# Arieys/MonteCarloPathTracing

Measured on AMD Instinct MI355X. Metric: Mrays/s on cornell-box 1280x720 SPP=256 (closest-hit queries actually traced / wall time incl. gather), higher is better.
Workload: dtype f64

## Files before the change

### montecarlopathtracing_amd/csrc/trace_pool.hpp

```cpp
#pragma once
#include "env.hpp"
#include "trace_persistent.hpp"
#include "vertex.hpp"

namespace mcpt {

struct NoPaths { static constexpr bool kPaths = false; };

#ifndef MCPT_POOL_WAVES
#define MCPT_POOL_WAVES 16
#endif
#ifndef MCPT_POOL_KT
#define MCPT_POOL_KT 20
#endif
#ifndef MCPT_POOL_STACK
#define MCPT_POOL_STACK 8
#endif
#define MCPT_POOL_SPILL (MCPT_FAST_STACK - MCPT_POOL_STACK)
#ifndef MCPT_POOL_CLAIMS
#define MCPT_POOL_CLAIMS 2
#endif
#define MCPT_POOL_CLAIM_ORDER __ATOMIC_ACQUIRE
#define MCPT_POOL_FILE_ORDER __ATOMIC_RELEASE

struct alignas(16) PoolOxy { double ox, oy; };
struct alignas(16) PoolOzDx { double oz, dx; };
struct alignas(16) PoolDyz { double dy, dz; };
struct alignas(16) PoolRcp { float rx, ry, rz, limit; };
typedef double pool_d2 __attribute__((ext_vector_type(2)));
template <class T>
__device__ __forceinline__ T pool_ld16(const T* p)
{
    static_assert(sizeof(T) == 16, "16-byte group");
    const pool_d2 v = *reinterpret_cast<const pool_d2*>(p);
    T r;
    __builtin_memcpy(&r, &v, 16);
    return r;
}

template <int NW, int KT, int SCAP>
struct PoolLds {
    PoolOxy oxy[KT * 64];
    PoolOzDx ozdx[KT * 64];
    PoolDyz dyz[KT * 64];
    PoolRcp rcp[KT * 64];
    double best_t[KT * 64];
    unsigned int q[KT * 64];
    int cur[KT * 64];
    int best_leaf[KT * 64];
    int spf[KT * 64];
    int stack[SCAP * KT * 64];
    unsigned int cls[5 * 64];
    unsigned int busy[64];
    int tbl[NW * 64];
    unsigned int stat[8];
    unsigned int live;
    unsigned int dry;
};

__device__ __forceinline__ int uni(int v) { return __builtin_amdgcn_readfirstlane(v); }
__device__ __forceinline__ long long uni(long long v)
{
    const int lo = __builtin_amdgcn_readfirstlane((int)(unsigned int)(unsigned long long)v);
    const int hi = __builtin_amdgcn_readfirstlane((int)(unsigned int)((unsigned long long)v >> 32));
    return (long long)(((unsigned long long)(unsigned int)hi << 32) | (unsigned int)lo);
}

template <class Src, int NW, int KT, int SCAP, class PP = NoPaths>
__device__ __forceinline__ void trace_pool(const DScene& S, const Src& src, TraceQueue* queue, long long* __restrict__ slow_list,
                                           unsigned int slow_cap, long long chunk, PoolLds<NW, KT, SCAP>& L, Work& w,
                                           int* __restrict__ spill ,
                                           const PP& pp = PP())
{
    static_assert(KT <= 32, "one 32-bit set per class");
    enum { C_INNER = 0, C_LEAF = 1, C_EXACT = 2, C_FIN = 3, C_SHADE = 4, C_DEAD = 5 };
    enum { F_FOUND = 256, F_AMBIG = 512, F_RAY = 1024, F_OWNFAIL = 2048  };
    const DFast& F = S.fast;
    const CwNode* __restrict__ nodes = F.cw;
    const DTri* __restrict__ tris = F.tris;
    const DTriPre* __restrict__ pre = F.pre;
    const TicketSchedule ts = make_ticket_schedule(src.total(), chunk);
    const int lane = threadIdx.x & 63, wave = uni((int)(threadIdx.x >> 6));
    const int stack_max = spill ? SCAP + MCPT_POOL_SPILL : SCAP;
    const int stack_cap = F.stack_cap < stack_max ? F.stack_cap : stack_max;
    int* __restrict__ my_spill = spill ? spill + (size_t)blockIdx.x * MCPT_POOL_SPILL * (KT * 64) : nullptr;
    auto st_put = [&](int e, int k, int v) __attribute__((always_inline)) {
        if (e < SCAP) L.stack[(e * KT + k) * 64 + lane] = v;
        else my_spill[((e - SCAP) * KT + k) * 64 + lane] = v;
    };
    auto st_get = [&](int e, int k) __attribute__((always_inline)) -> int {
        return e < SCAP ? L.stack[(e * KT + k) * 64 + lane] : my_spill[((e - SCAP) * KT + k) * 64 + lane];
    };

    for (int k = wave; k < KT; k += NW) { L.spf[k * 64 + lane] = 0; if constexpr (PP::kPaths) L.q[k * 64 + lane] = 0u; }
    int R = 1, NP = KT;
    if constexpr (PP::kPaths) { R = pp.nl + 1; NP = KT / R; }
    if (wave == 0) {
        L.cls[C_INNER * 64 + lane] = 0u; L.cls[C_LEAF * 64 + lane] = 0u; L.cls[C_EXACT * 64 + lane] = 0u;
        L.cls[C_FIN * 64 + lane] = PP::kPaths ? 0u : (unsigned int)((1ull << KT) - 1ull);
        L.cls[C_SHADE * 64 + lane] = PP::kPaths ? (unsigned int)((1ull << NP) - 1ull) : 0u;
        L.busy[lane] = 0u;
    }
    if (threadIdx.x == 0) { L.live = (PP::kPaths ? NP : KT) * 64; L.dry = 0; }
    if (threadIdx.x < 8) L.stat[threadIdx.x] = 0u;
    __syncthreads();

    unsigned int c_nodes = 0, c_rays = 0, c_exact = 0;
#ifdef MCPT_POOL_DEBUG
    unsigned long long d_used = 0, d_okc = 0, d_steps = 0, d_kill = 0, d_tickets = 0;
    unsigned long long d_cs[5] = {0, 0, 0, 0, 0}, d_cl[5] = {0, 0, 0, 0, 0}, d_sleep = 0, d_miss = 0, d_want[5] = {0, 0, 0, 0, 0};
    unsigned long long d_cyc[6] = {0, 0, 0, 0, 0, 0};
    unsigned long long d_t = __builtin_amdgcn_s_memtime();
    const unsigned long long d_t0 = d_t;
#endif
    long long next = 0, range_end = 0;
    bool queue_empty = false;
    int rot = wave % KT;
    const int rot_stride = (int)((0x13110d0bu >> (8 * ((wave >> 1) & 3))) & 255u) % KT | 1;
    const float s3f = __double2float_ru(3.0 * F.absmax), absmax_f = __double2float_ru(F.absmax);
    auto pad_of = [&](float of, float rf_) __attribute__((always_inline)) { return (0x1p-20f * 1.00001f) * ((fabsf(of) + s3f) * fabsf(rf_)); };
    auto margin_of = [&](const float of[3], const PoolRcp& a4) __attribute__((always_inline)) {
        const float rmax = fmaxf(fmaxf(fabsf(a4.rx), fabsf(a4.ry)), fabsf(a4.rz));
        const float scale = fmaxf(fmaxf(absmax_f, fabsf(of[0])), fmaxf(fabsf(of[1]), fabsf(of[2])));
        return rmax <= 0.99e6f ? (1.0000001e-9f * 1.00001f) * (scale * rmax) : __builtin_inff();
    };
    auto pop_next = [&](int idx, int k, int spf) __attribute__((always_inline)) -> int {
        int sp = spf & 255;
        if (sp == 0) return C_FIN;
        sp--;
        int nxt;
        if (!__ballot(sp >= SCAP)) { nxt = L.stack[(sp * KT + k) * 64 + lane]; __asm__ volatile("" : "+v"(nxt)); }
        else nxt = st_get(sp, k);
        const bool node = nxt >= 0;
        const int ref = -1 - nxt;
        const int first = node ? nxt : ref >> 4, cnt = (ref & 7) + 1;
        L.cur[idx] = first;
        L.spf[idx] = (spf & 0xff00) | sp | (node ? 0 : cnt << 16);
        return node ? C_INNER : C_LEAF;
    };

    for (;;) {
        const unsigned int m_inner = __hip_atomic_load(&L.cls[C_INNER * 64 + lane], __ATOMIC_RELAXED, __HIP_MEMORY_SCOPE_WORKGROUP);
        const unsigned int m_leaf = __hip_atomic_load(&L.cls[C_LEAF * 64 + lane], __ATOMIC_RELAXED, __HIP_MEMORY_SCOPE_WORKGROUP);
        const unsigned int m_exact = __hip_atomic_load(&L.cls[C_EXACT * 64 + lane], __ATOMIC_RELAXED, __HIP_MEMORY_SCOPE_WORKGROUP);
        const unsigned int m_fin = __hip_atomic_load(&L.cls[C_FIN * 64 + lane], __ATOMIC_RELAXED, __HIP_MEMORY_SCOPE_WORKGROUP);
        const int n_inner = __popcll(__ballot(m_inner != 0u));
        const int n_leaf = __popcll(__ballot(m_leaf != 0u));
        const int n_exact = __popcll(__ballot(m_exact != 0u));
        const bool fin_ok = PP::kPaths || !queue_empty || uni((int)__hip_atomic_load(&L.dry, __ATOMIC_RELAXED, __HIP_MEMORY_SCOPE_WORKGROUP)) == NW;
        const int n_fin = fin_ok ? __popcll(__ballot(m_fin != 0u)) : 0;
        unsigned int m_shade = 0u;
        int n_shade = 0;
        if constexpr (PP::kPaths) {
            m_shade = __hip_atomic_load(&L.cls[C_SHADE * 64 + lane], __ATOMIC_RELAXED, __HIP_MEMORY_SCOPE_WORKGROUP);
            n_shade = __popcll(__ballot(m_shade != 0u));
        }
        if (!(n_inner | n_leaf | n_exact | n_fin | n_shade)) {
            if (uni((int)__hip_atomic_load(&L.live, __ATOMIC_RELAXED, __HIP_MEMORY_SCOPE_WORKGROUP)) == 0) break;
            __builtin_amdgcn_s_sleep(4);
#ifdef MCPT_POOL_DEBUG
            d_sleep++;
#endif
            continue;
        }
        int c = C_FIN, best_score = n_fin;
        if (n_exact > best_score) { c = C_EXACT; best_score = n_exact; }
        if (n_leaf > best_score) { c = C_LEAF; best_score = n_leaf; }
        if (n_inner > best_score) { c = C_INNER; best_score = n_inner; }
        if (PP::kPaths && n_shade >= best_score && n_shade) { c = C_SHADE; best_score = n_shade; }
        c = uni(c);

        bool have = false;
        int k = 0;
        unsigned int cm = c == C_INNER ? m_inner : (c == C_LEAF ? m_leaf : (c == C_EXACT ? m_exact : (c == C_FIN ? m_fin : m_shade)));
        unsigned int* const cword = &L.cls[c * 64 + lane];
        const unsigned int below = 0xffffffffu >> (31 - rot), above = 0xffffffffu << rot;
#pragma unroll
        for (int attempt = 0; attempt < MCPT_POOL_CLAIMS; attempt++) {
            const bool want = !have && cm != 0u;
            if (attempt && !__ballot(want)) break;
            if (want) {
                int kk;
                if (wave & 1) { const unsigned int lo = cm & below; kk = 31 - __clz((int)(lo ? lo : cm)); }
                else { const unsigned int hi = cm & above; kk = __ffs((int)(hi ? hi : cm)) - 1; }
                const unsigned int bit = 1u << kk;
                const unsigned int old = __hip_atomic_fetch_and(cword, ~bit, MCPT_POOL_CLAIM_ORDER, __HIP_MEMORY_SCOPE_WORKGROUP);
                have = (old & bit) != 0u;
                k = kk;
                cm = old & ~bit;
            }
        }
        { rot += rot_stride; if (rot >= KT) rot -= KT; }
        const unsigned long long hv = __ballot(have);
#ifdef MCPT_POOL_DEBUG
        if (!hv) d_miss++;
#endif
        if (!hv) continue;
        const int n_have = __popcll(hv);
#ifdef MCPT_POOL_DEBUG
        { const unsigned long long tn = __builtin_amdgcn_s_memtime(); d_cyc[5] += tn - d_t; d_t = tn; }
        d_cs[c]++; d_cl[c] += n_have; d_want[c] += c == C_INNER ? n_inner : (c == C_LEAF ? n_leaf : (c == C_EXACT ? n_exact : (c == C_FIN ? n_fin : n_shade)));
#endif
        const int idx = k * 64 + lane;
        int nc = C_DEAD;
        __asm__ volatile("" ::: "memory");

        if (c == C_INNER) {
            bool refused = false;
            if (have) {
                const int cur = L.cur[idx];
                int spf = L.spf[idx];
                const PoolOxy a0 = pool_ld16(&L.oxy[idx]); const PoolOzDx a1 = pool_ld16(&L.ozdx[idx]); const PoolRcp a4 = L.rcp[idx];
                const float limit = a4.limit;
                RayF rf;
                rf.o[0] = (float)a0.ox; rf.o[1] = (float)a0.oy; rf.o[2] = (float)a1.oz;
                rf.r[0] = a4.rx; rf.r[1] = a4.ry; rf.r[2] = a4.rz;
                rf.pad[0] = pad_of(rf.o[0], a4.rx); rf.pad[1] = pad_of(rf.o[1], a4.ry); rf.pad[2] = pad_of(rf.o[2], a4.rz);
                int sp = spf & 255;
                if (sp > stack_cap - 3) {
                    L.spf[idx] = spf | F_AMBIG; nc = C_FIN; refused = true;
                } else {
                    const CwHits h = cw_step(nodes + cur, rf, limit);
                    const int n_hit = (h.ref[0] != MCPT_FAST_EMPTY) + (h.ref[1] != MCPT_FAST_EMPTY) + (h.ref[2] != MCPT_FAST_EMPTY) + (h.ref[3] != MCPT_FAST_EMPTY);
                    if (!__ballot(sp + n_hit - 1 > SCAP)) {
                        int* const col = &L.stack[k * 64 + lane];
                        if (n_hit >= 4) col[sp * (KT * 64)] = h.ref[3];
                        if (n_hit >= 3) col[(sp + n_hit - 3) * (KT * 64)] = h.ref[2];
                        if (n_hit >= 2) col[(sp + n_hit - 2) * (KT * 64)] = h.ref[1];
                        sp += n_hit > 1 ? n_hit - 1 : 0;
                    } else {
                        if (h.ref[3] != MCPT_FAST_EMPTY) { st_put(sp, k, h.ref[3]); sp++; }
                        if (h.ref[2] != MCPT_FAST_EMPTY) { st_put(sp, k, h.ref[2]); sp++; }
                        if (h.ref[1] != MCPT_FAST_EMPTY) { st_put(sp, k, h.ref[1]); sp++; }
                    }
                    int nxt = h.ref[0];
                    {
                        const bool pop = nxt == MCPT_FAST_EMPTY && sp > 0;
                        if (pop) sp--;
                        if (!__ballot(pop && sp >= SCAP)) { if (pop) { nxt = L.stack[(sp * KT + k) * 64 + lane]; __asm__ volatile("" : "+v"(nxt)); } }
                        else if (pop) nxt = st_get(sp, k);
                    }
                    const bool node = nxt >= 0, none = nxt == MCPT_FAST_EMPTY;
                    const int ref = -1 - nxt;
                    const int first = node ? nxt : ref >> 4, cnt = (ref & 7) + 1;
                    if (!none) L.cur[idx] = first;
                    spf = (spf & 0xff00) | sp | ((!node && !none) ? cnt << 16 : 0);
                    L.spf[idx] = spf;
                    nc = node ? C_INNER : (none ? C_FIN : C_LEAF);
                }
            }
            c_nodes += (unsigned int)(n_have - __popcll(__ballot(refused)));
        } else if (c == C_LEAF) {
            if (have) {
                const int cur = L.cur[idx];
                const int spf0 = L.spf[idx];
                const int cnt = (spf0 >> 16) & 255;
                const PoolOxy a0 = pool_ld16(&L.oxy[idx]); const PoolOzDx a1 = pool_ld16(&L.ozdx[idx]); const PoolDyz a2 = pool_ld16(&L.dyz[idx]); const PoolRcp a4 = L.rcp[idx];
                const float of[3] = {(float)a0.ox, (float)a0.oy, (float)a1.oz};
                const float limit = a4.limit, margin = margin_of(of, a4);
                unsigned int surv = 0;
                w.tris += cnt;
                if (!pre) surv = (1u << cnt) - 1u;
                else {
                    Ray r; r.o = mk(a0.ox, a0.oy, a1.oz); r.d = mk(a1.dx, a2.dy, a2.dz);
                    const PreRay pr = make_pre_ray(F, r, of, margin);
                    surv = leaf_survivors(pre, cur, cnt, pr, limit);
#ifdef MCPT_PRE_CHECK
                    const unsigned int wrong = leaf_wrongly_rejected(tris, cur, cnt, surv, r, (spf0 & F_FOUND) != 0, L.best_t[idx]);
                    w.pre_wrong += (unsigned int)__popc(wrong); surv |= wrong;
#endif
                }
                if (surv) { L.spf[idx] = (spf0 & 0xffff) | ((int)surv << 16); nc = C_EXACT; }
                else nc = pop_next(idx, k, spf0);
            }
        } else if (c == C_EXACT) {
            c_exact += (unsigned int)n_have;
            if (have) {
                const int cur = L.cur[idx];
                int spf = L.spf[idx];
                int surv = (spf >> 16) & 255;
                const PoolOxy a0 = pool_ld16(&L.oxy[idx]); const PoolOzDx a1 = pool_ld16(&L.ozdx[idx]); const PoolDyz a2 = pool_ld16(&L.dyz[idx]);
                const double best_t = L.best_t[idx];
                Ray r; r.o = mk(a0.ox, a0.oy, a1.oz); r.d = mk(a1.dx, a2.dy, a2.dz);
                const int kk = __ffs(surv) - 1;
                surv &= surv - 1;
                const int ti = cur + kk;
                const DTri* tr = tris + ti;
                const bool found = (spf & F_FOUND) != 0;
                V3 p;
                const bool hit = tri_hit(tr, r, p);
                if (hit) {
                    const double ta = (p.x - r.o.x) * fast_rcp(r.d.x);
                    if (ta > 0.0) {
                        const double band = best_t * 0x1p-47;
                        if (!found || ta < best_t - band) {
                            const PoolRcp a4 = L.rcp[idx];
                            const float of[3] = {(float)a0.ox, (float)a0.oy, (float)a1.oz};
                            L.best_t[idx] = ta; L.best_leaf[idx] = ti;
                            L.rcp[idx].limit = lead_limit(ta, margin_of(of, a4));
                            const bool own = own_box_hit(tr, r, mk(fast_rcp(r.d.x), fast_rcp(r.d.y), fast_rcp(r.d.z)));
                            spf = (spf & ~F_OWNFAIL) | F_FOUND | (own ? 0 : F_OWNFAIL);
                        } else if (!(ta > best_t + band)) {
                            const DTri* lt = tris + L.best_leaf[idx];
                            if (tie_prefers_new(r, p.x, hit_point(lt, r).x, tr, lt)) {
                                L.best_t[idx] = ta; L.best_leaf[idx] = ti;
                                const bool own = own_box_hit(tr, r, mk(fast_rcp(r.d.x), fast_rcp(r.d.y), fast_rcp(r.d.z)));
                                spf = (spf & ~F_OWNFAIL) | (own ? 0 : F_OWNFAIL);
                            }
                        }
                    }
                }
                if (surv) {
                    spf = (spf & 0xffff) | (surv << 16);
                    L.spf[idx] = spf; nc = C_EXACT;
                }
                else nc = pop_next(idx, k, spf);
                if (nc == C_FIN) L.spf[idx] = spf & 0xffff;
            }
        } else if (PP::kPaths && c == C_FIN) {
            if constexpr (PP::kPaths) {
                if (have) {
                    const int spf = L.spf[idx];
                    const PoolOxy a0 = pool_ld16(&L.oxy[idx]); const PoolOzDx a1 = pool_ld16(&L.ozdx[idx]); const PoolDyz a2 = pool_ld16(&L.dyz[idx]);
                    Ray r; r.o = mk(a0.ox, a0.oy, a1.oz); r.d = mk(a1.dx, a2.dy, a2.dz);
                    bool found = (spf & F_FOUND) != 0;
                    bool ambiguous = (spf & F_AMBIG) != 0;
                    int leaf_ref = -1, mat = -1;
                    if (found) {
                        const DTri* tr = tris + L.best_leaf[idx];
                        if (spf & F_OWNFAIL) ambiguous = true;
                        leaf_ref = tr->leaf; mat = tr->material;
                    }
                    if (ambiguous) {
                        Hit hh;
                        Work w2 = {0, 0};
                        const bool ok = fast_path_ok(F, r) ? trace_lane_fast(S, r, hh, w2, pp.lane_stack(wave, lane), 1) : trace_closest(S, r, hh, w2);
                        w.nodes += w2.nodes; w.tris += w2.tris;
                        found = ok; leaf_ref = ok ? hh.leaf : -1; mat = ok ? S.tris[hh.leaf].material : -1;
                    }
                    L.best_leaf[idx] = found ? leaf_ref : -1;
                    L.cur[idx] = found ? mat : -1;
                    const unsigned int bit = 1u << k;
                    const unsigned int old = __hip_atomic_fetch_and(&L.busy[lane], ~bit, __ATOMIC_ACQ_REL, __HIP_MEMORY_SCOPE_WORKGROUP);
                    const int pk = (int)(((float)k + 0.5f) * pp.inv_r);
                    const unsigned int pm = ((1u << R) - 1u) << (pk * R);
                    if (((old & ~bit) & pm) == 0u)
                        __hip_atomic_fetch_or(&L.cls[C_SHADE * 64 + lane], 1u << pk, MCPT_POOL_FILE_ORDER, __HIP_MEMORY_SCOPE_WORKGROUP);
                    nc = C_DEAD;
                }
            }
        } else if (PP::kPaths) {
            if constexpr (PP::kPaths) {
                const WfArgs& a = pp.a;
                const int nl = pp.nl;
                const auto [nplanes, nlights, folded] = path_lights<PP::kEnv, PP::kPick>(S, nl);
                const long long cap = a.cap;
                const int s0 = k * R;
                const size_t plane = (size_t)pp.npc * 64;
                double* __restrict__ rd = pp.recd + (size_t)blockIdx.x * (size_t)(9 + 3 * nl) * plane + (size_t)k * 64 + lane;
                int* __restrict__ ri = pp.reci + (size_t)blockIdx.x * (size_t)(3 + nl) * plane + (size_t)k * 64 + lane;
                enum { P_FREE = 0, P_ADOPTED = 1, P_VERTEX = 2 };
                enum { RI_ID = 0, RI_DEPTH = 1, RI_BT = 2, RI_EXPECT = 3 };
                enum { RD_T = 0, RD_L = 3, RD_W = 6, RD_C = 9 };
                auto ldp = [&](int f) __attribute__((always_inline)) { return mk(rd[(size_t)f * plane], rd[(size_t)(f + 1) * plane], rd[(size_t)(f + 2) * plane]); };
                auto stp = [&](int f, const V3& v) __attribute__((always_inline)) { rd[(size_t)f * plane] = v.x; rd[(size_t)(f + 1) * plane] = v.y; rd[(size_t)(f + 2) * plane] = v.z; };
                int mode = have ? (int)L.q[s0 * 64 + lane] : P_FREE;
                int id = 0, leaf = -1, in_type = RT_TRANSMISSION;
                uint32_t depth = 0;
                V3 T = mk(1, 1, 1), Lr = mk(0, 0, 0), p = mk(0, 0, 0), dir = mk(0, 0, 0);
                bool at_vertex = false;
                if (have && mode != P_FREE) {
                    id = ri[RI_ID * plane]; depth = (uint32_t)ri[RI_DEPTH * plane];
                    const int bt = ri[RI_BT * plane];
                    T = ldp(RD_T); Lr = ldp(RD_L);
                    V3 L_dir = mk(0, 0, 0);
                    for (int l = 0; l < nl; l++) {
                        const int expect = ri[(size_t)(RI_EXPECT + l) * plane];
                        if (expect == -2) continue;
                        const V3 cc = ldp(RD_C + 3 * l);
                        add_if_visible(L_dir, cc, L.cur[(s0 + l) * 64 + lane] == expect);
                    }
                    if (mode == P_ADOPTED && folded) Lr = Lr + L_dir;
                    else Lr = Lr + mul(T, L_dir);
                    const int bidx = (s0 + nl) * 64 + lane;
                    const int hl = bt >= 0 ? L.best_leaf[bidx] : -1;
                    if (hl >= 0) {
                        if (!(mode == P_ADOPTED && folded)) T = after_bounce(T, ldp(RD_W));
                        const PoolOxy b0 = pool_ld16(&L.oxy[bidx]); const PoolOzDx b1 = pool_ld16(&L.ozdx[bidx]); const PoolDyz b2 = pool_ld16(&L.dyz[bidx]);
                        Ray br; br.o = mk(b0.ox, b0.oy, b1.oz); br.d = mk(b1.dx, b2.dy, b2.dz);
                        p = hit_point(S.tris + hl, br); dir = neg(br.d); in_type = bt & 7; depth++; leaf = hl;
                        at_vertex = true;
                    } else if (PP::kEnv && bt >= 0) {
                        const V3 Tn = (mode == P_ADOPTED && folded) ? T : after_bounce(T, ldp(RD_W));
                        const PoolOzDx b1 = pool_ld16(&L.ozdx[bidx]); const PoolDyz b2 = pool_ld16(&L.dyz[bidx]);
                        Lr = env_escape(S.env, Lr, Tn, bt, mk(b1.dx, b2.dy, b2.dz));
                    }
                }
                bool ended = have && mode != P_FREE && !at_vertex;
                const DMaterial* m = nullptr;
                V3 pn = mk(0, 0, 0), kd = mk(0, 0, 0);
                const int n_shades = __popcll(__ballot(at_vertex));
                const unsigned int deepest = wave_max(at_vertex ? depth : 0u);
                if (at_vertex) {
                    m = S.materials + S.tris[leaf].material;
                    if (m->light >= 0) {
                        const V3 rad = ld3(S.lights[m->light].radiance);
                        if (depth == 0) Lr = rad;
                        else if (in_type != RT_DIFFUSE) Lr = Lr + mul(T, rad);
                        ended = true; at_vertex = false;
                    } else vertex_surface(S, leaf, p, m, pn, kd);
                }
                if (ended) { a.rad[(size_t)id * 3] = Lr.x; a.rad[(size_t)id * 3 + 1] = Lr.y; a.rad[(size_t)id * 3 + 2] = Lr.z; mode = P_FREE; }
                unsigned int nb_inner = 0u, nb_fin = 0u;
                auto emit = [&](int sk, const V3& o, const V3& d) __attribute__((always_inline)) {
                    const int i2 = sk * 64 + lane;
                    Ray r; r.o = o; r.d = d;
                    const bool okf = fast_path_ok(F, r);
                    const V3 rcp = mk(fast_rcp(d.x), fast_rcp(d.y), fast_rcp(d.z));
                    PoolOxy b0; b0.ox = o.x; b0.oy = o.y;
                    PoolOzDx b1; b1.oz = o.z; b1.dx = d.x;
                    PoolDyz b2; b2.dy = d.y; b2.dz = d.z;
                    PoolRcp b4; b4.rx = (float)rcp.x; b4.ry = (float)rcp.y; b4.rz = (float)rcp.z; b4.limit = __builtin_inff();
                    L.oxy[i2] = b0; L.ozdx[i2] = b1; L.dyz[i2] = b2; L.rcp[i2] = b4;
                    L.best_t[i2] = 0;
                    L.cur[i2] = 0; L.best_leaf[i2] = -1; L.spf[i2] = okf ? F_RAY : (F_RAY | F_AMBIG);
                    if (okf) nb_inner |= 1u << sk; else nb_fin |= 1u << sk;
                };
                int n_shadow = 0, n_skipped = 0, n_bounce = 0;
                if (at_vertex) {
                    const RngKey key = sample_key(a, id);
                    int sample_mat = -1;
                    for (int l = 0; l < nplanes; l++) {
                        V3 direction, cc;
                        const int expect = PP::kPick ? light_sample_one<PP::kPick>(S, key, depth, p, pn, kd, direction, cc) : light_sample(S, key, depth, l, p, pn, kd, sample_mat, direction, cc);
                        ri[(size_t)(RI_EXPECT + l) * plane] = expect;
                        if (expect != -2) { stp(RD_C + 3 * l, cc); emit(s0 + l, p + direction * 0.01, direction); n_shadow++; }
                        else n_skipped++;
                    }
                    if constexpr (PP::kEnv) {
                        V3 direction, cc;
                        const int expect = env_light_sample(S.env, key, depth, (uint32_t)nlights, pn, kd, direction, cc);
                        ri[(size_t)(RI_EXPECT + nplanes) * plane] = expect;
                        if (expect != -2) { stp(RD_C + 3 * nplanes, cc); emit(s0 + nplanes, p + direction * 0.01, direction); n_shadow++; }
                    }
                    V3 nd = mk(0, 0, 0), wgt = mk(1, 1, 1);
                    const int bt = bounce_sample(key, depth, nlights, m, dir, pn, kd, nd, wgt);
                    ri[RI_BT * plane] = bt;
                    if (bt >= 0) { stp(RD_W, wgt); emit(s0 + nl, (bt & MCPT_BT_NO_OFFSET) ? p : p + nd * 0.01, nd); n_bounce++; }
                    ri[RI_DEPTH * plane] = (int)depth;
                    stp(RD_T, T); stp(RD_L, Lr);
                    mode = P_VERTEX;
                }
                const bool want_path = have && mode == P_FREE;
                const unsigned long long wb = __ballot(want_path);
                bool dead = false;
                if (wb) {
                    long long mine = pp.n;
                    if (!queue_empty) {
                        const unsigned int want = (unsigned int)__popcll(wb);
                        unsigned int got = 0;
                        if (lane == 0) got = atomicAdd(&a.counts->finish_claimed, want);
                        got = (unsigned int)uni((int)got);
                        if ((long long)got + want >= pp.n) queue_empty = true;
                        mine = (long long)got + (int)__builtin_amdgcn_mbcnt_hi((unsigned int)(wb >> 32), __builtin_amdgcn_mbcnt_lo((unsigned int)wb, 0u));
                    }
                    if (want_path) {
                        if (mine < pp.n) {
                            const long long j = mine;
                            id = a.out.id[j];
                            depth = (uint32_t)a.depth;
                            T = mk(1, 1, 1); Lr = mk(0, 0, 0);
                            if (folded && a.depth == 0) { const int b0 = a.out.btype[j]; if (b0 >= 0) T = first_vertex_throughput(S, a, id, b0); }
                            else if (a.depth > 0 || folded) T = ldc(a.out.T, cap, j);
                            if (a.depth > 0) Lr = ldc(a.out.L, cap, j);
                            if (a.depth == 0) { const PrimaryHit* ph = a.hits + (a.first_slot + id / a.spp); p = mk(ph->p[0], ph->p[1], ph->p[2]); }
                            else p = ldc(a.out.p, cap, j);
                            for (int l = 0; l < nl; l++) {
                                const int expect = a.out.expect[(long long)l * cap + j];
                                ri[(size_t)(RI_EXPECT + l) * plane] = expect;
                                if (expect != -2) {
                                    const V3 cc = ldc(a.out.c + (long long)l * 3 * cap, cap, j), d = ldc(a.rays.d + (long long)l * 3 * cap, cap, j);
                                    stp(RD_C + 3 * l, cc); emit(s0 + l, p + d * 0.01, d);
                                }
                            }
                            const int bt = a.out.btype[j];
                            ri[RI_BT * plane] = bt;
                            if (bt >= 0) {
                                const V3 bd = ldc(a.out.bdir, cap, j);
                                if (!folded) stp(RD_W, ldc(a.out.w, cap, j));
                                emit(s0 + nl, (bt & MCPT_BT_NO_OFFSET) ? p : p + bd * 0.01, bd);
                            }
                            ri[RI_ID * plane] = id; ri[RI_DEPTH * plane] = (int)depth;
                            stp(RD_T, T); stp(RD_L, Lr);
                            mode = P_ADOPTED;
                        } else dead = true;
                    }
                }
                if (have) {
                    L.q[s0 * 64 + lane] = (unsigned int)mode;
                    const unsigned int nb = nb_inner | nb_fin;
                    if (nb) __hip_atomic_fetch_or(&L.busy[lane], nb, __ATOMIC_RELAXED, __HIP_MEMORY_SCOPE_WORKGROUP);
                    if (nb_inner) __hip_atomic_fetch_or(&L.cls[C_INNER * 64 + lane], nb_inner, MCPT_POOL_FILE_ORDER, __HIP_MEMORY_SCOPE_WORKGROUP);
                    if (nb_fin) __hip_atomic_fetch_or(&L.cls[C_FIN * 64 + lane], nb_fin, MCPT_POOL_FILE_ORDER, __HIP_MEMORY_SCOPE_WORKGROUP);
                    nc = (mode != P_FREE && !nb) ? C_SHADE : C_DEAD;
                    w.rays += (unsigned int)__popc(nb);
                }
                const int n_dead = __popcll(__ballot(have && dead));
                if (n_dead && lane == 0) __hip_atomic_fetch_sub(&L.live, (unsigned int)n_dead, __ATOMIC_RELAXED, __HIP_MEMORY_SCOPE_WORKGROUP);
                const unsigned int t_sh = (unsigned int)wave_sum((unsigned long long)n_shadow), t_sk = (unsigned int)wave_sum((unsigned long long)n_skipped),
                                   t_bo = (unsigned int)wave_sum((unsigned long long)n_bounce);
                if (lane == 0) {
                    if (n_shades) atomicAdd(&L.stat[0], (unsigned int)n_shades);
                    if (t_sh) atomicAdd(&L.stat[1], t_sh);
                    if (t_bo) atomicAdd(&L.stat[2], t_bo);
                    if (t_sk) atomicAdd(&L.stat[3], t_sk);
                    if (deepest) atomicMax(&L.stat[4], deepest);
                }
            }
        } else {
            if (have) {
                const int spf = L.spf[idx];
                if (spf & F_RAY) {
                    const PoolOxy a0 = pool_ld16(&L.oxy[idx]); const PoolOzDx a1 = pool_ld16(&L.ozdx[idx]); const PoolDyz a2 = pool_ld16(&L.dyz[idx]);
                    const long long slot = (long long)L.q[idx];
                    Ray r; r.o = mk(a0.ox, a0.oy, a1.oz); r.d = mk(a1.dx, a2.dy, a2.dz);
                    const bool found = (spf & F_FOUND) != 0;
                    bool ambiguous = (spf & F_AMBIG) != 0;
                    Hit h; h.leaf = -1; h.t = 0; h.p = mk(0, 0, 0);
                    if (found) {
                        const DTri* tr = tris + L.best_leaf[idx];
                        if (spf & F_OWNFAIL) ambiguous = true;
                        h.leaf = tr->leaf;
                        h.mat = tr->material;
                        h.p = hit_point(tr, r);
                        h.t = (h.p.x - r.o.x) / r.d.x;
                    }
                    if (ambiguous) defer_ray(queue, slow_list, slow_cap, slot, true);
                    else src.store(slot, found, h);
                }
            }
            bool got = false;
            bool all_dry = queue_empty;
            if (!queue_empty && next >= range_end) {
                unsigned long long tk = 0;
                if (lane == 0) tk = atomicAdd(&queue->head, 1ull);
                const bool in_range = ticket_range(ts, uni((long long)tk), next, range_end);
#ifdef MCPT_POOL_DEBUG
                d_tickets++;
#endif
                if (!in_range) {
                    queue_empty = true;
                    unsigned int before = 0;
                    if (lane == 0) before = __hip_atomic_fetch_add(&L.dry, 1u, __ATOMIC_RELAXED, __HIP_MEMORY_SCOPE_WORKGROUP);
                    all_dry = uni((int)before) + 1 == NW;
                }
            }
            if (!queue_empty) {
                const long long left = range_end - next;
                const int avail = left < 64 ? (int)left : 64;
                Ray nr; nr.o = mk(0, 0, 0); nr.d = mk(1, 1, 1);
                const bool valid = lane < avail && src.fetch(next + lane, nr);
                const bool ok = valid && fast_path_ok(F, nr);
                const unsigned long long V = __ballot(ok);
                const int n_ok = __popcll(V);
                const int rank_ok = (int)__builtin_amdgcn_mbcnt_hi((unsigned int)(V >> 32), __builtin_amdgcn_mbcnt_lo((unsigned int)V, 0u));
                int used = avail;
                if (n_ok > n_have) used = __ffsll((long long)__ballot(ok && rank_ok == n_have - 1));
                used = uni(used);
                if (valid && !ok && lane < used) defer_ray(queue, slow_list, slow_cap, next + lane, false);
                if (ok && rank_ok < n_have) L.tbl[wave * 64 + rank_ok] = lane;
                const int rank_need = (int)__builtin_amdgcn_mbcnt_hi((unsigned int)(hv >> 32), __builtin_amdgcn_mbcnt_lo((unsigned int)hv, 0u));
                got = have && rank_need < n_ok;
                __asm__ volatile("" ::: "memory");
                const int from = got ? L.tbl[wave * 64 + rank_need] : lane;
                Ray r;
                r.o.x = __shfl(nr.o.x, from, 64); r.o.y = __shfl(nr.o.y, from, 64); r.o.z = __shfl(nr.o.z, from, 64);
                r.d.x = __shfl(nr.d.x, from, 64); r.d.y = __shfl(nr.d.y, from, 64); r.d.z = __shfl(nr.d.z, from, 64);
                if (got) {
                    const V3 rcp = mk(fast_rcp(r.d.x), fast_rcp(r.d.y), fast_rcp(r.d.z));
                    PoolOxy b0; b0.ox = r.o.x; b0.oy = r.o.y;
                    PoolOzDx b1; b1.oz = r.o.z; b1.dx = r.d.x;
                    PoolDyz b2; b2.dy = r.d.y; b2.dz = r.d.z;
                    PoolRcp b4; b4.rx = (float)rcp.x; b4.ry = (float)rcp.y; b4.rz = (float)rcp.z; b4.limit = __builtin_inff();
                    L.oxy[idx] = b0; L.ozdx[idx] = b1; L.dyz[idx] = b2; L.rcp[idx] = b4;
                    L.best_t[idx] = 0;
                    L.cur[idx] = 0; L.best_leaf[idx] = -1; L.spf[idx] = F_RAY;
                    L.q[idx] = (unsigned int)(next + from);
                    nc = C_INNER;
                }
                next += used;
#ifdef MCPT_POOL_DEBUG
                d_used += used; d_okc += __popcll(__ballot(ok && lane < used)); d_steps++;
#endif
                c_rays += (unsigned int)__popcll(__ballot(got));
            }
            if (have && !got) {
                if (queue_empty && all_dry) nc = C_DEAD;
                else { L.spf[idx] = 0; nc = C_FIN; }
            }
            const int n_dead = __popcll(__ballot(have && nc == C_DEAD));
#ifdef MCPT_POOL_DEBUG
            d_kill += n_dead;
#endif
            if (n_dead && lane == 0) __hip_atomic_fetch_sub(&L.live, (unsigned int)n_dead, __ATOMIC_RELAXED, __HIP_MEMORY_SCOPE_WORKGROUP);
        }
        __asm__ volatile("" ::: "memory");
#ifdef MCPT_POOL_DEBUG
        { const unsigned long long tn = __builtin_amdgcn_s_memtime(); d_cyc[c] += tn - d_t; d_t = tn; }
#endif
        if (have && nc != C_DEAD)
            __hip_atomic_fetch_or(&L.cls[nc * 64 + lane], 1u << k, MCPT_POOL_FILE_ORDER, __HIP_MEMORY_SCOPE_WORKGROUP);
    }
    if (lane == 0) { w.nodes += c_nodes; w.rays += c_rays; w.exact += c_exact; }
#ifdef MCPT_POOL_DEBUG
    if constexpr (PP::kPaths) {
        if (lane == 0 && pp.a.ctr) {
            PoolAccount& o = pp.a.ctr->dbg.account;
            for (int i = 0; i < 5; i++) { atomicAdd(&o.steps[i], d_cs[i]); atomicAdd(&o.lanes[i], d_cl[i]); atomicAdd(&o.cycles[i], d_cyc[i]); }
            atomicAdd(&o.sleeps, d_sleep); atomicAdd(&o.missed, d_miss); atomicAdd(&o.overhead, d_cyc[5]);
            atomicAdd(&o.life, __builtin_amdgcn_s_memtime() - d_t0); atomicAdd(&o.waves, 1ull);
        }
    } else
    if (lane == 0 && w.dbg) {
        {
            PoolAccount& o = w.dbg->account;
            for (int i = 0; i < 4; i++) { atomicAdd(&o.steps[i], d_cs[i]); atomicAdd(&o.lanes[i], d_cl[i]); atomicAdd(&o.cycles[i], d_cyc[i]); }
            atomicAdd(&o.sleeps, d_sleep); atomicAdd(&o.missed, d_miss); atomicAdd(&o.overhead, d_cyc[5]);
            atomicAdd(&o.life, __builtin_amdgcn_s_memtime() - d_t0); atomicAdd(&o.waves, 1ull);
        }
        PoolDebug& g = w.dbg->pool;
        atomicAdd(&g.used, d_used); atomicAdd(&g.ok, d_okc); atomicAdd(&g.refills, d_steps); atomicAdd(&g.retired, d_kill); atomicAdd(&g.tickets, d_tickets);
        atomicAdd(&g.started, (unsigned long long)c_rays);
        for (int i = 0; i < 4; i++) { atomicAdd(&g.class_steps[i], d_cs[i]); atomicAdd(&g.class_lanes[i], d_cl[i]); atomicAdd(&g.class_want[i], d_want[i]); }
        atomicAdd(&g.sleeps, d_sleep); atomicAdd(&g.missed, d_miss);
        if (threadIdx.x == 0 && blockIdx.x == 0) { atomicAdd(&g.slots, (unsigned long long)ts.total); atomicAdd(&g.launches, 1ull); }
    }
#endif
}

}
```

Measured before the change: 5406.

## Split leaf triangle testing into pair-sized steps in the pooled traversal scheduler

Leaf triangle work is now processed at most two triangles per C_LEAF step instead of the whole leaf at once. A ray slot with more triangles left re-enters the leaf class with an advanced cursor, instead of popping the stack. The per-slot state word is repacked through new helper functions. These encode the remaining count, a begun flag and a 2-bit survivor mask. The intent is to even out per-step work across lanes and shrink the survivor state, at the cost of more scheduler iterations and class switches per leaf.

```diff
diff --git a/montecarlopathtracing_amd/csrc/pool_slot_words.hpp b/montecarlopathtracing_amd/csrc/pool_slot_words.hpp
--- /dev/null
+++ b/montecarlopathtracing_amd/csrc/pool_slot_words.hpp
@@ -0,0 +1,35 @@
+#pragma once
+
+namespace mcpt {
+
+#ifdef __HIPCC__
+#define MCPT_SPF_FN __host__ __device__ __forceinline__ constexpr
+#else
+#define MCPT_SPF_FN inline constexpr
+#endif
+
+enum : int { SPF_FOUND = 256, SPF_AMBIG = 512, SPF_RAY = 1024, SPF_OWNFAIL = 2048 };
+enum : int { SPF_STACK_MASK = 0xff, SPF_FLAG_MASK = 0xf00, SPF_PAIR_SHIFT = 16, SPF_REST_SHIFT = 18, SPF_REST_MASK = 15, SPF_BEGUN = 1 << 22 };
+
+MCPT_SPF_FN int spf_stack(int spf) { return spf & SPF_STACK_MASK; }
+MCPT_SPF_FN int spf_flags(int spf) { return spf & SPF_FLAG_MASK; }
+MCPT_SPF_FN int spf_pair(int spf) { return (spf >> SPF_PAIR_SHIFT) & 3; }
+MCPT_SPF_FN int spf_rest(int spf) { return (spf >> SPF_REST_SHIFT) & SPF_REST_MASK; }
+MCPT_SPF_FN bool spf_begun(int spf) { return (spf & SPF_BEGUN) != 0; }
+
+MCPT_SPF_FN int spf_walk(int spf) { return spf & (SPF_STACK_MASK | SPF_FLAG_MASK); }
+MCPT_SPF_FN int spf_node(int spf, int sp) { return spf_flags(spf) | sp; }
+MCPT_SPF_FN int spf_leaf(int spf, int sp, int count) { return spf_flags(spf) | sp | (count << SPF_REST_SHIFT); }
+MCPT_SPF_FN int spf_pair_size(int spf) { return spf_rest(spf) < 2 ? spf_rest(spf) : 2; }
+MCPT_SPF_FN int spf_tested(int spf, int survivors)
+{
+    return spf_walk(spf) | SPF_BEGUN | ((spf_rest(spf) - spf_pair_size(spf)) << SPF_REST_SHIFT) | ((survivors & 3) << SPF_PAIR_SHIFT);
+}
+MCPT_SPF_FN int spf_with_pair(int spf, int survivors) { return (spf & ~(3 << SPF_PAIR_SHIFT)) | ((survivors & 3) << SPF_PAIR_SHIFT); }
+
+enum : int { SPF_NEXT_PAIR = 0, SPF_POP = 1 };
+MCPT_SPF_FN int spf_after_pair(int spf) { return spf_rest(spf) > 0 ? SPF_NEXT_PAIR : SPF_POP; }
+
+#undef MCPT_SPF_FN
+
+}
diff --git a/montecarlopathtracing_amd/csrc/trace_pool.hpp b/montecarlopathtracing_amd/csrc/trace_pool.hpp
--- a/montecarlopathtracing_amd/csrc/trace_pool.hpp
+++ b/montecarlopathtracing_amd/csrc/trace_pool.hpp
@@ -1,5 +1,6 @@
 #pragma once
 #include "env.hpp"
+#include "pool_slot_words.hpp"
 #include "trace_persistent.hpp"
 #include "vertex.hpp"
 
@@ -74,7 +75,7 @@
 {
     static_assert(KT <= 32, "one 32-bit set per class");
     enum { C_INNER = 0, C_LEAF = 1, C_EXACT = 2, C_FIN = 3, C_SHADE = 4, C_DEAD = 5 };
-    enum { F_FOUND = 256, F_AMBIG = 512, F_RAY = 1024, F_OWNFAIL = 2048  };
+    enum { F_FOUND = SPF_FOUND, F_AMBIG = SPF_AMBIG, F_RAY = SPF_RAY, F_OWNFAIL = SPF_OWNFAIL  };
     const DFast& F = S.fast;
     const CwNode* __restrict__ nodes = F.cw;
     const DTri* __restrict__ tris = F.tris;
@@ -125,7 +126,7 @@
         return rmax <= 0.99e6f ? (1.0000001e-9f * 1.00001f) * (scale * rmax) : __builtin_inff();
     };
     auto pop_next = [&](int idx, int k, int spf) __attribute__((always_inline)) -> int {
-        int sp = spf & 255;
+        int sp = spf_stack(spf);
         if (sp == 0) return C_FIN;
         sp--;
         int nxt;
@@ -135,7 +136,7 @@
         const int ref = -1 - nxt;
         const int first = node ? nxt : ref >> 4, cnt = (ref & 7) + 1;
         L.cur[idx] = first;
-        L.spf[idx] = (spf & 0xff00) | sp | (node ? 0 : cnt << 16);
+        L.spf[idx] = node ? spf_node(spf, sp) : spf_leaf(spf, sp, cnt);
         return node ? C_INNER : C_LEAF;
     };
 
@@ -216,7 +217,7 @@
                 rf.o[0] = (float)a0.ox; rf.o[1] = (float)a0.oy; rf.o[2] = (float)a1.oz;
                 rf.r[0] = a4.rx; rf.r[1] = a4.ry; rf.r[2] = a4.rz;
                 rf.pad[0] = pad_of(rf.o[0], a4.rx); rf.pad[1] = pad_of(rf.o[1], a4.ry); rf.pad[2] = pad_of(rf.o[2], a4.rz);
-                int sp = spf & 255;
+                int sp = spf_stack(spf);
                 if (sp > stack_cap - 3) {
                     L.spf[idx] = spf | F_AMBIG; nc = C_FIN; refused = true;
                 } else {
@@ -244,7 +245,7 @@
                     const int ref = -1 - nxt;
                     const int first = node ? nxt : ref >> 4, cnt = (ref & 7) + 1;
                     if (!none) L.cur[idx] = first;
-                    spf = (spf & 0xff00) | sp | ((!node && !none) ? cnt << 16 : 0);
+                    spf = (!node && !none) ? spf_leaf(spf, sp, cnt) : spf_node(spf, sp);
                     L.spf[idx] = spf;
                     nc = node ? C_INNER : (none ? C_FIN : C_LEAF);
                 }
@@ -254,12 +255,12 @@
             if (have) {
                 const int cur = L.cur[idx];
                 const int spf0 = L.spf[idx];
-                const int cnt = (spf0 >> 16) & 255;
+                const int cnt = spf_pair_size(spf0);
                 const PoolOxy a0 = pool_ld16(&L.oxy[idx]); const PoolOzDx a1 = pool_ld16(&L.ozdx[idx]); const PoolDyz a2 = pool_ld16(&L.dyz[idx]); const PoolRcp a4 = L.rcp[idx];
                 const float of[3] = {(float)a0.ox, (float)a0.oy, (float)a1.oz};
                 const float limit = a4.limit, margin = margin_of(of, a4);
                 unsigned int surv = 0;
-                w.tris += cnt;
+                if (!spf_begun(spf0)) w.tris += spf_rest(spf0);
                 if (!pre) surv = (1u << cnt) - 1u;
                 else {
                     Ray r; r.o = mk(a0.ox, a0.oy, a1.oz); r.d = mk(a1.dx, a2.dy, a2.dz);
@@ -270,15 +271,17 @@
                     w.pre_wrong += (unsigned int)__popc(wrong); surv |= wrong;
 #endif
                 }
-                if (surv) { L.spf[idx] = (spf0 & 0xffff) | ((int)surv << 16); nc = C_EXACT; }
-                else nc = pop_next(idx, k, spf0);
+                const int spf = spf_tested(spf0, (int)surv);
+                if (surv) { L.spf[idx] = spf; nc = C_EXACT; }
+                else if (spf_after_pair(spf) == SPF_NEXT_PAIR) { L.cur[idx] = cur + 2; L.spf[idx] = spf; nc = C_LEAF; }
+                else nc = pop_next(idx, k, spf);
             }
         } else if (c == C_EXACT) {
             c_exact += (unsigned int)n_have;
             if (have) {
                 const int cur = L.cur[idx];
                 int spf = L.spf[idx];
-                int surv = (spf >> 16) & 255;
+                int surv = spf_pair(spf);
                 const PoolOxy a0 = pool_ld16(&L.oxy[idx]); const PoolOzDx a1 = pool_ld16(&L.ozdx[idx]); const PoolDyz a2 = pool_ld16(&L.dyz[idx]);
                 const double best_t = L.best_t[idx];
                 Ray r; r.o = mk(a0.ox, a0.oy, a1.oz); r.d = mk(a1.dx, a2.dy, a2.dz);
@@ -310,12 +313,11 @@
                         }
                     }
                 }
-                if (surv) {
-                    spf = (spf & 0xffff) | (surv << 16);
-                    L.spf[idx] = spf; nc = C_EXACT;
-                }
+                spf = spf_with_pair(spf, surv);
+                if (surv) { L.spf[idx] = spf; nc = C_EXACT; }
+                else if (spf_after_pair(spf) == SPF_NEXT_PAIR) { L.cur[idx] = cur + 2; L.spf[idx] = spf; nc = C_LEAF; }
                 else nc = pop_next(idx, k, spf);
-                if (nc == C_FIN) L.spf[idx] = spf & 0xffff;
+                if (nc == C_FIN) L.spf[idx] = spf_walk(spf);
             }
         } else if (PP::kPaths && c == C_FIN) {
             if constexpr (PP::kPaths) {
```

Result: faster. 5495 (median of 6 runs) (+1.6%).
